# RQLuo/CDLNet-video

Hardware: AMD Instinct MI355X
Metric: Mpix/s denoised (fwd+bwd) at K=30,M=64,P=7 (higher is better)
Workload: dtype f32 (split-bf16 x3 MFMA, fp32 accumulate, fp32 storage)

## Files before the change

### cdlnet-video_amd/csrc/cdl_fused2d.hip

```cpp
#include <atomic>
#include <cstdlib>
#include <type_traits>
#include <mutex>
#include <utility>
#include <vector>

#include "cdl_common.h"

#ifdef CDL_F2D_WY4
#define CDL_WY 4
#define cdl_fused2d_assemble cdl_fused2d_assemble_wy4
#define cdl_fused2d_backward cdl_fused2d_backward_wy4
#define cdl_fused2d_code_bytes cdl_fused2d_code_bytes_wy4
#define cdl_fused2d_dtau_reduce cdl_fused2d_dtau_reduce_wy4
#define cdl_fused2d_forward cdl_fused2d_forward_wy4
#define cdl_fused2d_frag_bytes cdl_fused2d_frag_bytes_wy4
#define cdl_fused2d_iter_fwd cdl_fused2d_iter_fwd_wy4
#define cdl_fused2d_map_words cdl_fused2d_map_words_wy4
#define cdl_fused2d_patch_floats cdl_fused2d_patch_floats_wy4
#define cdl_fused2d_prep cdl_fused2d_prep_wy4
#define cdl_fused2d_stage_bwd cdl_fused2d_stage_bwd_wy4
#define cdl_fused2d_support_map cdl_fused2d_support_map_wy4
#define cdl_fused2d_supported cdl_fused2d_supported_wy4
#define cdl_fused2d_tiles cdl_fused2d_tiles_wy4
// ... 928 lines not shown
            ws |= (zz != 0.0f ? 1u : 0u) << (16 * R + v);
            wg |= (__builtin_bit_cast(unsigned, zz) >> 31) << (16 * R + v);
        }
    map[((size_t)n * 4 + 2 * h) * HW + pix] = ws;
    map[((size_t)n * 4 + 2 * h + 1) * HW + pix] = wg;
}

struct WgradParams {
    const float *X[2];
    const float *T[2];
    float *partial;
    int N, H, W, tilesX, tilesY, numTiles;
    int rev;
    int single;
};

template <int MT, int PREC, int LAY>
__global__ __launch_bounds__(512) void k_wgrad2d(WgradParams p)
{
    extern __shared__ __attribute__((aligned(16))) unsigned char dsm[];
    __bf16 *thin = reinterpret_cast<__bf16 *>(dsm);
    __bf16 *imgs = reinterpret_cast<__bf16 *>(dsm + WG_THIN_BYTES);
    constexpr int M = 32 * MT;
    const int tid = threadIdx.x, lane = tid & 63, wid = tid >> 6;
    const int op = wid >> 2, wq = wid & 3;
    const int wxi = wq & 1, wyi = wq >> 1;
    const int c = lane & 31, h = lane >> 5;
    const size_t HW = (size_t)p.H * p.W;
    __bf16 *wimg = imgs + (size_t)wid * (MT * 2) * IMG_ELEMS;
    f32x16 acc[MT][2];
#pragma unroll
    for (int R = 0; R < MT; ++R)
#pragma unroll
        for (int tt = 0; tt < 2; ++tt)
#pragma unroll
            for (int v = 0; v < 16; ++v) acc[R][tt][v] = 0.0f;

    for (int i = tid; i < WG_THIN_BYTES / 16; i += 512) reinterpret_cast<uint4 *>(dsm)[i] = make_uint4(0, 0, 0, 0);

    const bool present = p.X[op] != nullptr;
    const int nsteps = p.single ? (p.numTiles + 1) / 2 : p.numTiles;
    for (int t0 = blockIdx.x; t0 < nsteps; t0 += gridDim.x) {
        const int t = p.single ? 2 * t0 + op : t0;
        const bool active = present && t < p.numTiles;
        int bid = p.rev ? p.numTiles - 1 - t : t;
        const int txi = bid % p.tilesX; bid /= p.tilesX;
        const int tyi = bid % p.tilesY;
        const int n = active ? bid / p.tilesY : 0;
        const int tx0 = txi * TW, ty0 = tyi * GW_TH;
        __syncthreads();
        if (active) {
            const float *timg = p.T[op] + (size_t)n * HW;
            constexpr int NSW = (GW_RTH * RTW + 255) / 256;
            float tv[NSW];
#pragma unroll
            for (int k = 0; k < NSW; ++k) {
                const int i = (tid & 255) + k * 256;
                const int yy = i / RTW, xx = i % RTW;
                const int gy = ty0 - HALO + yy, gx = tx0 - HALO + xx;
                const bool ok = i < GW_RTH * RTW && gy >= 0 && gy < p.H && gx >= 0 && gx < p.W;
                const float v = timg[ok ? (size_t)gy * p.W + gx : 0];
                tv[k] = ok ? v : 0.0f;
            }
#pragma unroll
            for (int k = 0; k < NSW; ++k) {
                const int i = (tid & 255) + k * 256;
                if (i >= GW_RTH * RTW) continue;
                const int yy = i / RTW, xx = i % RTW;
                const __bf16 hh = (__bf16)tv[k];
                const __bf16 ll = (__bf16)(tv[k] - (float)hh);
#pragma unroll
                for (int s = 0; s < 4; ++s)
                    if (xx - s >= 0) {
                        thin[((op * 2 + 0) * 4 + s) * TCOPY + yy * TPITCH + xx - s] = hh;
                        if (PREC != 1) thin[((op * 2 + 1) * 4 + s) * TCOPY + yy * TPITCH + xx - s] = ll;
                    }
            }
        }
        __syncthreads();
        if (!active) continue;

        const int x = tx0 + wxi * 32 + c;
        const bool xok = x < p.W;
#pragma unroll 1
        for (int b = 0; b < RB; ++b) {
            const int yl = wyi * RB + b, y = ty0 + yl;
            const bool valid = xok && y < p.H;
            const size_t img_b = lay_image_bytes<LAY>(M, p.H, p.W);
            const __amdgpu_buffer_rsrc_t rs = uniform_rsrc((const char *)p.X[op] + (size_t)n * img_b, img_b);
            const int voff = valid ? (int)((4 * h) * HW + (size_t)y * p.W + x) * 4 : OOB;
            const int hw4 = (int)HW * 4;
            float xv[MT][16];
            u32x2 xr[MT][4];
            if (LAY == LAY_BLK16) {
                const int XB = (p.W + 31) / 32, xb = (tx0 >> 5) + wxi;
                blk16_load_raw<MT>(xr, rs, valid ? ((y * XB + xb) * (M / 4) * 32 + h * 32 + c) * 8 : OOB);
            } else if (LAY == LAY_BLK) {
                const int XB = (p.W + 31) / 32, xb = (tx0 >> 5) + wxi;
                blk_load<LAY_BLK, MT>(xv, rs, valid ? ((y * XB + xb) * (M / 4) * 32 + h * 32 + c) * 16 : OOB);
            } else {
#pragma unroll
                for (int R = 0; R < MT; ++R)
#pragma unroll
                    for (int v = 0; v < 16; ++v)
                        xv[R][v] = buf_ld(rs, voff, (32 * R + 8 * (v >> 2) + (v & 3)) * hw4);
            }
#pragma unroll
            for (int R = 0; R < MT; ++R)
#pragma unroll
                for (int qv = 0; qv < 4; ++qv) {
                    bf16x4 hi4, lo4;
                    if (LAY == LAY_BLK16) {
                        hi4 = __builtin_bit_cast(bf16x4, xr[R][qv]);
                    } else {
#pragma unroll
                        for (int e = 0; e < 4; ++e) {
                            const float val = xv[R][4 * qv + e];
                            const __bf16 hh = (__bf16)val;
                            hi4[e] = hh;
                            lo4[e] = (__bf16)(val - (float)hh);
                        }
                    }
                    const int slot = (2 * qv + h) ^ ((c >> 1) & 7);
                    __bf16 *dst = wimg + (size_t)(R * 2) * IMG_ELEMS + c * 32 + slot * 4;
                    *reinterpret_cast<bf16x4 *>(dst) = hi4;
                    if (PREC != 1 && LAY != LAY_BLK16) *reinterpret_cast<bf16x4 *>(dst + IMG_ELEMS) = lo4;
                }
            __builtin_amdgcn_fence(__ATOMIC_RELEASE, "wavefront");
            __builtin_amdgcn_wave_barrier();
#pragma unroll
            for (int kk = 0; kk < 2; ++kk) {
                bf16x8 Bh[2], Bl[2];
#pragma unroll
                for (int tt = 0; tt < 2; ++tt) {
                    const int tap = 32 * tt + c, ti = tap >> 3, tj = tap & 7;
                    const int e0 = wxi * 32 + 16 * kk + 8 * h + (tj & 4);
                    const __bf16 *ph = thin + ((op * 2 + 0) * 4 + (tj & 3)) * TCOPY + (yl + ti) * TPITCH + e0;
                    const bf16x4 a0 = *reinterpret_cast<const bf16x4 *>(ph);
                    const bf16x4 a1 = *reinterpret_cast<const bf16x4 *>(ph + 4);
                    Bh[tt] = __builtin_shufflevector(a0, a1, 0, 1, 2, 3, 4, 5, 6, 7);
                    if (PREC != 1) {
                        const __bf16 *pl = ph + 4 * TCOPY;
                        const bf16x4 b0 = *reinterpret_cast<const bf16x4 *>(pl);
                        const bf16x4 b1 = *reinterpret_cast<const bf16x4 *>(pl + 4);
                        Bl[tt] = __builtin_shufflevector(b0, b1, 0, 1, 2, 3, 4, 5, 6, 7);
                    }
                }
#pragma unroll
                for (int R = 0; R < MT; ++R) {
                    const int gg = (lane >> 4) & 1, qq = (lane >> 2) & 3, pp = lane & 3;
                    bf16x4 part[2][2];
#pragma unroll
                    for (int half = 0; half < 2; ++half) {
                        const int row = 16 * kk + 8 * h + 4 * half + qq;
                        const int slot = (4 * gg + pp) ^ ((row >> 1) & 7);
                        const __bf16 *src = wimg + (size_t)(R * 2) * IMG_ELEMS + row * 32 + slot * 4;
                        part[0][half] = __builtin_amdgcn_ds_read_tr16_b64_v4bf16(
                            (__attribute__((address_space(3))) bf16x4 *)(src));
                        if (PREC != 1 && LAY != LAY_BLK16)
                            part[1][half] = __builtin_amdgcn_ds_read_tr16_b64_v4bf16(
                                (__attribute__((address_space(3))) bf16x4 *)(src + IMG_ELEMS));
                    }
                    const bf16x8 Ah = __builtin_shufflevector(part[0][0], part[0][1], 0, 1, 2, 3, 4, 5, 6, 7);
                    bf16x8 Al;
                    if (PREC != 1 && LAY != LAY_BLK16) Al = __builtin_shufflevector(part[1][0], part[1][1], 0, 1, 2, 3, 4, 5, 6, 7);
#pragma unroll
                    for (int tt = 0; tt < 2; ++tt) {
                        if (PREC != 1) {
                            if (LAY != LAY_BLK16) acc[R][tt] = __builtin_amdgcn_mfma_f32_32x32x16_bf16(Al, Bh[tt], acc[R][tt], 0, 0, 0);
                            acc[R][tt] = __builtin_amdgcn_mfma_f32_32x32x16_bf16(Ah, Bl[tt], acc[R][tt], 0, 0, 0);
                            if (PREC == 2 && LAY != LAY_BLK16) acc[R][tt] = __builtin_amdgcn_mfma_f32_32x32x16_bf16(Al, Bl[tt], acc[R][tt], 0, 0, 0);
                        }
                        acc[R][tt] = __builtin_amdgcn_mfma_f32_32x32x16_bf16(Ah, Bh[tt], acc[R][tt], 0, 0, 0);
                    }
                }
            }
            __builtin_amdgcn_fence(__ATOMIC_RELEASE, "wavefront");
            __builtin_amdgcn_wave_barrier();
        }
    }

    float *red = reinterpret_cast<float *>(dsm);
    for (int w = 0; w < 4; ++w) {
        __syncthreads();
        if (wq == w) {
#pragma unroll
            for (int R = 0; R < MT; ++R)
#pragma unroll
                for (int tt = 0; tt < 2; ++tt)
#pragma unroll
                    for (int v = 0; v < 16; ++v) {
                        const int ch = 32 * R + (v & 3) + 8 * (v >> 2) + 4 * h;
                        float *dstw = &red[(op * M + ch) * 64 + 32 * tt + c];
                        *dstw = (w == 0 ? 0.0f : *dstw) + acc[R][tt][v];
                    }
        }
    }
    __syncthreads();
    float *dst = p.partial + (size_t)blockIdx.x * 2 * M * 64;
    for (int i = tid; i < 2 * M * 64; i += 512) dst[i] = red[i];
}

__global__ __launch_bounds__(1024) void k_wgrad_reduce(const float *__restrict__ partial, int G,
                                                       float *__restrict__ dw0, float alpha0,
                                                       float *__restrict__ dw1, float alpha1, int M, int P, int merge = 0)
{
    __shared__ float red[32][33];
    const int o = threadIdx.x & 31, part = threadIdx.x >> 5;
    const int t = blockIdx.x * 32 + o;
    const int per = M * P * P;
    const bool live = t < (merge ? per : 2 * per);
    float sum = 0.0f;
    int op = 0, r = 0;
    if (live) {
        op = t / per; r = t % per;
        const int ch = r / (P * P), ij = r % (P * P), off = (7 - P) / 2;
        const int tap = 8 * (ij / P + off) + (ij % P + off);
        for (int g = part; g < G; g += 32) {
            sum += partial[((size_t)(g * 2 + op) * M + ch) * 64 + tap];
            if (merge) sum += partial[((size_t)(g * 2 + 1) * M + ch) * 64 + tap];
        }
    }
    red[part][o] = sum;
    __syncthreads();
    if (part == 0 && live) {
        float *dw = op ? dw1 : dw0;
        if (dw) {
            float tot = 0.0f;
#pragma unroll
            for (int k = 0; k < 32; ++k) tot += red[k][o];
            dw[r] = (op ? alpha1 : alpha0) * tot;
        }
    }
}

__global__ __launch_bounds__(1024) void k_dtau_reduce(const float *__restrict__ partial,
                                                      const float *__restrict__ c, float *__restrict__ dt0,
                                                      float *__restrict__ dt1, int N, int per_img, int M)
{
    __shared__ float r0[256][4], r1[256][4];
    const int mi = threadIdx.x & 3, part = threadIdx.x >> 2;
    const int m = blockIdx.x * 4 + mi;
    float a0 = 0.0f, a1 = 0.0f;
    const int rows = N * per_img;
    if (m < M)
        for (int row = part; row < rows; row += 256) {
            const float v = partial[(size_t)row * M + m];
            a0 += v;
            if (c) a1 = fmaf(c[row / per_img], v, a1);
        }
    r0[part][mi] = a0;
    r1[part][mi] = a1;
    __syncthreads();
    for (int stride = 128; stride >= 1; stride >>= 1) {
        if (part < stride) { r0[part][mi] += r0[part + stride][mi]; r1[part][mi] += r1[part + stride][mi]; }
        __syncthreads();
    }
    if (part == 0 && m < M) { dt0[m] = r0[0][mi]; dt1[m] = r1[0][mi]; }
}

inline hipStream_t S(void *s) { return reinterpret_cast<hipStream_t>(s); }

inline bool fused_shape_ok(const cdl_geom *g)
{
    if (!cdl_geom_ok(g)) return false;
    if (g->C != 1 || g->D != 1 || g->Pd != 1 || g->sd != 1 || g->sh != 1 || g->sw != 1) return false;
    if (g->Ph != g->Pw || g->Ph > 7 || (g->Ph & 1) == 0 || g->ph != g->Ph / 2 || g->pw != g->Pw / 2) return false;
    if (g->M != 32 && g->M != 64) return false;
    if (blk_image_elems(g->M, g->H, g->W) * 4 >= ((size_t)1 << 31)) return false;
    return true;
}

inline int debug_flags() { return cdl_opts().fused_debug; }

inline int tiles_x(const cdl_geom *g) { return (g->W + TW - 1) / TW; }
inline int tiles_y(const cdl_geom *g) { return (g->H + TH - 1) / TH; }

struct Flags {
    int prec, rev, lin, lout;
    bool ok;
};
// ... 58 lines not shown
{
    const size_t tiles = (size_t)p.N * p.tilesX * p.tilesY;
    size_t cus = (size_t)cdl_cu_count();
    const int cap = cdl_opts().fused_grid;
    if (cap > 0 && (size_t)cap < cus) cus = (size_t)cap;
    return (int)(tiles < cus ? tiles : cus);
}

int dispatch_stage(const cdl_geom *g, const FusedParams &p, int mode, const Flags &f, hipStream_t st)
{
    dim3 grid((unsigned)stage_grid(g, p));
    if (g->M == 64)
        return f.prec == 0   ? launch_stage<2, 0>(p, mode, f.lin, f.lout, grid, st)
               : f.prec == 1 ? launch_stage<2, 1>(p, mode, f.lin, f.lout, grid, st)
                             : launch_stage<2, 2>(p, mode, f.lin, f.lout, grid, st);
    return f.prec == 0   ? launch_stage<1, 0>(p, mode, f.lin, f.lout, grid, st)
           : f.prec == 1 ? launch_stage<1, 1>(p, mode, f.lin, f.lout, grid, st)
                         : launch_stage<1, 2>(p, mode, f.lin, f.lout, grid, st);
}

int wgrad_grid(const cdl_geom *g)
{
    const size_t tiles = (size_t)g->N * tiles_x(g) * ((g->H + GW_TH - 1) / GW_TH);
    return (int)(tiles < 512 ? tiles : 512);
}

template <int MT, int PREC, int LAY>
int launch_wgrad_one(const WgradParams &p, int G, hipStream_t st)
{
    const size_t lds = (size_t)WG_THIN_BYTES + (size_t)8 * MT * 2 * IMG_ELEMS * 2;
    if (int rc = cdl_ensure_dynamic_lds((const void *)k_wgrad2d<MT, PREC, LAY>, (int)lds)) return rc;
    k_wgrad2d<MT, PREC, LAY><<<G, 512, lds, st>>>(p);
    hipError_t e = hipGetLastError();
    return e == hipSuccess ? 0 : -(int)e;
}

template <int MT, int PREC>
int launch_wgrad(const WgradParams &p, int lay, int G, hipStream_t st)
{
    if (lay == LAY_BLK) return launch_wgrad_one<MT, PREC, LAY_BLK>(p, G, st);
    if (lay == LAY_BLK16) return launch_wgrad_one<MT, PREC, LAY_BLK16>(p, G, st);
    return launch_wgrad_one<MT, PREC, LAY_NCHW>(p, G, st);
}

}

extern "C" {

// ... 64 lines not shown
    k_support_map<<<(unsigned)((total + 255) / 256), 256, 0, S(stream)>>>(z, map, g->N, g->M, g->H, g->W);
    CDL_LAUNCH_CHECK();
    return 0;
}

int cdl_fused2d_iter_fwd(const cdl_geom *g, const float *r, const float *zin, const float *tau,
                         const void *frags, float sgn, float *zout, float *patches, unsigned *map_out,
                         int precision, void *stream)
{
    if (!fused_shape_ok(g)) return CDL_EUNSUPPORTED;
    if (!r || !tau || !frags || !zout || !patches || zout == zin) return CDL_EINVAL;
    const Flags f = parse_flags(precision);
    if (!f.ok) return CDL_EINVAL;
    FusedParams p = {};
    p.rev = f.rev;
    p.r = r; p.zin = zin; p.zout = zout; p.tau = tau; p.map = map_out;
    p.frags = reinterpret_cast<const uint4 *>(frags);
    p.patches = patches; p.sgn = sgn; p.do_synth = 1; CDL_DBG_FIELD(p.dbg = debug_flags();)
    p.N = g->N; p.H = g->H; p.W = g->W;
    p.tilesX = tiles_x(g); p.tilesY = tiles_y(g);
    return dispatch_stage(g, p, zin ? MODE_FWD : MODE_FIRST, f, S(stream));
}

static int stage_bwd(const cdl_geom *g, const float *thin, const float *base, const unsigned *map, const void *frags,
                     float *du_out, float *patches, float *dtau_partial, int do_synth, int precision, const float *r2,
                     float alpha, float *dA, float *workspace, void *stream)
{
    if (!fused_shape_ok(g)) return CDL_EUNSUPPORTED;
    if (!thin || !map || !frags || !du_out || !dtau_partial || du_out == base) return CDL_EINVAL;
    if (do_synth && !patches) return CDL_EINVAL;
    if (r2 && (!dA || !workspace)) return CDL_EINVAL;
    const Flags f = parse_flags(precision);
    if (!f.ok) return CDL_EINVAL;
    FusedParams p = {};
    p.rev = f.rev;
    p.r = thin; p.zin = base; p.map = const_cast<unsigned *>(map); p.zout = du_out; p.dtau = dtau_partial;
    p.frags = reinterpret_cast<const uint4 *>(frags);
    p.patches = patches; p.sgn = 1.0f; p.do_synth = do_synth ? 1 : 0; CDL_DBG_FIELD(p.dbg = debug_flags();)
    p.N = g->N; p.H = g->H; p.W = g->W;
    p.tilesX = tiles_x(g); p.tilesY = tiles_y(g);
    p.r2 = r2; p.da_partial = workspace;
    int rc = dispatch_stage(g, p, MODE_BWD, f, S(stream));
    if (rc || !r2) return rc;
    const int G = stage_grid(g, p);
    const int total = 2 * g->M * g->Ph * g->Pw;
    k_wgrad_reduce<<<(total + 31) / 32, 1024, 0, S(stream)>>>(workspace, G, dA, alpha, nullptr, 0.0f, g->M, g->Ph);
    CDL_LAUNCH_CHECK();
    return 0;
}

int cdl_fused2d_stage_bwd(const cdl_geom *g, const float *thin, const float *base, const unsigned *map,
                          const void *frags, float *du_out, float *patches, float *dtau_partial, int do_synth,
                          const float *r2, float alpha, float *dA, float *workspace, int precision, void *stream)
{
    if (!r2 != !dA || !r2 != !workspace) return CDL_EINVAL;
    return stage_bwd(g, thin, base, map, frags, du_out, patches, dtau_partial, do_synth, precision, r2, alpha, dA, workspace,
                     stream);
}

int cdl_fused2d_dtau_reduce(const cdl_geom *g, const float *dtau_partial, const float *c, float *dt0, float *dt1,
                            float *dtau_n, void *stream)
{
    if (!fused_shape_ok(g)) return CDL_EUNSUPPORTED;
    if (!dtau_partial || !dt0 || !dt1) return CDL_EINVAL;
    const int per_img = tiles_x(g) * tiles_y(g);
    k_dtau_reduce<<<(g->M + 3) / 4, 1024, 0, S(stream)>>>(dtau_partial, c, dt0, dt1, g->N, per_img, g->M);
    CDL_LAUNCH_CHECK();
    if (!dtau_n) return 0;
    return cdl_dtau_per_sample(dtau_partial, g->N, g->M, per_img, (size_t)per_img * g->M, 1, g->M, dtau_n, stream);
}

size_t cdl_fused2d_wgrad_workspace_floats(const cdl_geom *g)
{
    if (!fused_shape_ok(g)) return 0;
    const size_t own = (size_t)wgrad_grid(g) * 2 * g->M * 64;
#ifndef CDL_F2D_WY4
    return larger(own, cdl_fused2d_wgrad_workspace_floats_wy4(g));
#else
    return own;
#endif
}

int cdl_fused2d_wgrad(const cdl_geom *g, const float *X0, const float *T0, float alpha0, float *dw0,
                      const float *X1, const float *T1, float alpha1, float *dw1, float *workspace,
                      int precision, void *stream)
{
    if (!fused_shape_ok(g)) return CDL_EUNSUPPORTED;
    if (!workspace || (!X0 && !X1)) return CDL_EINVAL;
    if ((X0 && (!T0 || !dw0)) || (X1 && (!T1 || !dw1))) return CDL_EINVAL;
    const Flags f = parse_flags(precision);
    if (!f.ok) return CDL_EINVAL;
    WgradParams p = {};
    p.rev = f.rev;
    p.X[0] = X0; p.T[0] = T0; p.X[1] = X1; p.T[1] = T1;
    p.single = (X0 != nullptr) != (X1 != nullptr);
    if (p.single) {
        if (!X0) { X0 = X1; T0 = T1; alpha0 = alpha1; dw0 = dw1; X1 = nullptr; }
        p.X[0] = p.X[1] = X0; p.T[0] = p.T[1] = T0;
    }
    p.partial = workspace;
    p.N = g->N; p.H = g->H; p.W = g->W;
    p.tilesX = tiles_x(g); p.tilesY = (g->H + GW_TH - 1) / GW_TH;
    p.numTiles = p.N * p.tilesX * p.tilesY;
    int G = wgrad_grid(g);
    if (p.single && G > (p.numTiles + 1) / 2) G = (p.numTiles + 1) / 2;
    int rc;
    if (g->M == 64)
        rc = f.prec == 0 ? launch_wgrad<2, 0>(p, f.lin, G, S(stream))
             : f.prec == 1 ? launch_wgrad<2, 1>(p, f.lin, G, S(stream)) : launch_wgrad<2, 2>(p, f.lin, G, S(stream));
    else
        rc = f.prec == 0 ? launch_wgrad<1, 0>(p, f.lin, G, S(stream))
             : f.prec == 1 ? launch_wgrad<1, 1>(p, f.lin, G, S(stream)) : launch_wgrad<1, 2>(p, f.lin, G, S(stream));
    if (rc) return rc;
    const int total = 2 * g->M * g->Ph * g->Pw;
    k_wgrad_reduce<<<(total + 31) / 32, 1024, 0, S(stream)>>>(workspace, G, X0 ? dw0 : nullptr, alpha0,
                                                             X1 ? dw1 : nullptr, alpha1, g->M, g->Ph, p.single);
    CDL_LAUNCH_CHECK();
    return 0;
}

int cdl_fused2d_assemble(const cdl_geom *g, const float *patches, const float *mask, const float *sub,
                         float alpha, float *out, float *acc, int acc_add, void *stream)
{
    if (!fused_shape_ok(g)) return CDL_EUNSUPPORTED;
    if (!patches || (!out && !acc)) return CDL_EINVAL;
    if ((size_t)g->N * g->H * g->W >= ((size_t)1 << 20) && (g->W & 3) == 0 && !cdl_opts().scalar_assemble) {
        dim3 grid((unsigned)((g->W + 255) / 256), (unsigned)((g->H + 7) / 8), (unsigned)g->N);
        k_assemble_v4<<<grid, 256, 0, S(stream)>>>(patches, mask, sub, alpha, out, g->N, g->H, g->W, tiles_x(g), tiles_y(g), acc, acc_add);
    } else if ((size_t)g->N * g->H * g->W >= ((size_t)1 << 20)) {
        dim3 grid((unsigned)((g->W + 255) / 256), (unsigned)((g->H + 3) / 4), (unsigned)g->N);
        k_assemble<4><<<grid, 256, 0, S(stream)>>>(patches, mask, sub, alpha, out, g->N, g->H, g->W, tiles_x(g), tiles_y(g), acc, acc_add);
    } else {
        dim3 grid((unsigned)((g->W + 255) / 256), (unsigned)g->H, (unsigned)g->N);
        k_assemble<1><<<grid, 256, 0, S(stream)>>>(patches, mask, sub, alpha, out, g->N, g->H, g->W, tiles_x(g), tiles_y(g), acc, acc_add);
    }
    CDL_LAUNCH_CHECK();
    return 0;
}

}

// ... 170 lines not shown
    if (K < 1 || !yp || !wA || !wB || !z || !maps || !g_xp || !dA || !dB || !dt || !du0 || !du1 || !q || !frags ||
        !patches || !dtau_partial || !wgrad_ws || (K > 1 && !r))
        return CDL_EINVAL;
    const int M = g->M;
    float *du[2] = {du0, du1};
    const Flags f = parse_flags(precision);
    if (!f.ok || f.lout != 0) return CDL_EINVAL;
    const int L = f.lin;
#ifndef CDL_F2D_WY4
    if (L == LAY_BLK16)
        return cdl_fused2d_backward_wy4(g, K, yp, mask, c, wA, wB, z, r, maps, g_xp, g_z, dA, dB, dt, du0, du1, q, frags,
                                        patches, dtau_partial, wgrad_ws, precision, dyp, dtau, stream);
#endif
    const int sdir = snake_enabled() ? (((K - 1) & 1) ? CDL_TILES_REVERSED : 0) : 0;
    const int wdir = snake_enabled() ? (sdir ^ CDL_TILES_REVERSED) : 0;
    const int sprec = f.prec | sdir, wprec = f.prec | wdir;
    int rc = cdl_fused2d_wgrad(g, z[K - 1], g_xp, 1.0f, dB[0], nullptr, nullptr, 0.0f, nullptr, wgrad_ws,
                               wprec, stream);
    if (rc) return rc;
    const float *thin = g_xp, *base = g_z;
    const size_t fb = cdl_fused2d_frag_bytes(M);
    rc = prep_pairs(wB, wA, K, 0, frags, M, g->Ph, S(stream));
    if (rc) return rc;
    for (int k = K - 1, flip = 0; k >= 0; --k, flip ^= 1) {
        const void *fk = static_cast<const char *>(frags) + (size_t)k * fb;
        float *duk = du[flip];
        const bool ride = TH == GW_TH && cdl_opts().fused_da;
        {
            TimingScope ts(1, S(stream));
            rc = stage_bwd(g, thin, base, maps[k], fk, duk, patches, dtau_partial, k >= 1 || dyp,
                           sprec | CDL_LAYOUT_IN(k == K - 1 ? LAY_NCHW : L) | CDL_LAYOUT_OUT(L),
                           ride ? (k >= 1 ? r[k - 1] : yp) : nullptr, k >= 1 ? -1.0f : 1.0f, dA[k], wgrad_ws, stream);
        }
        if (rc) return rc;
        rc = cdl_fused2d_dtau_reduce(g, dtau_partial, c, dt + (size_t)k * 2 * M, dt + (size_t)k * 2 * M + M,
                                     dtau ? dtau + (size_t)k * g->N * M : nullptr, stream);
        if (rc) return rc;
        if (k == 0 && dyp) {
            rc = cdl_fused2d_assemble(g, patches, nullptr, nullptr, 1.0f, nullptr, dyp, K > 1, stream);
            if (rc) return rc;
        }
        if (k >= 1) {
            rc = cdl_fused2d_assemble(g, patches, mask, nullptr, -1.0f, q, dyp, k < K - 1, stream);
            if (rc) return rc;
            {
                TimingScope ts(2, S(stream));
                rc = ride ? cdl_fused2d_wgrad(g, z[k - 1], q, 1.0f, dB[k], nullptr, nullptr, 0.0f, nullptr, wgrad_ws,
                                              wprec | CDL_LAYOUT_IN(L), stream)
                          : cdl_fused2d_wgrad(g, duk, r[k - 1], -1.0f, dA[k], z[k - 1], q, 1.0f, dB[k], wgrad_ws,
                                              wprec | CDL_LAYOUT_IN(L), stream);
            }
            thin = q;
        } else if (!ride) {
            rc = cdl_fused2d_wgrad(g, duk, yp, 1.0f, dA[0], nullptr, nullptr, 0.0f, nullptr, wgrad_ws,
                                   wprec | CDL_LAYOUT_IN(L), stream);
        }
        if (rc) return rc;
        base = duk;
    }
    return 0;
}

}
```

### cdlnet-video_amd/ops.py

```python
import ctypes
from dataclasses import dataclass
from typing import Optional, Tuple

import torch

from . import _lib


def _stream():
    return ctypes.c_void_p(torch.cuda.current_stream().cuda_stream)


def _first_cuda_tensor(args, kwargs=None):
    for a in list(args) + (list(kwargs.values()) if kwargs else []):
        if torch.is_tensor(a):
            if a.is_cuda:
                return a
        elif isinstance(a, (list, tuple)):
            t = _first_cuda_tensor(a)
            if t is not None:
                return t
    return None


# ... 626 lines not shown
                                          float(alpha), _ptr(dA), _ptr(workspace), flags, _stream())
    _lib.check(rc, "cdl_fused2d_stage_bwd")
    return out if dA is None else (out, dA)


def fused_dtau_reduce(g: Geometry, dtau_partial, c, dt_k, dtau_n=None):
    assert dt_k.is_contiguous() and dt_k.numel() == 2 * g.M
    assert dtau_n is None or (dtau_n.is_contiguous() and dtau_n.numel() == g.N * g.M)
    gs = g.c_struct()
    base = dt_k.data_ptr()
    rc = _lib.lib().cdl_fused2d_dtau_reduce(ctypes.byref(gs), _ptr(dtau_partial), _ptr(_opt(c, "c")),
                                            ctypes.c_void_p(base), ctypes.c_void_p(base + 4 * g.M), _ptr(dtau_n),
                                            _stream())
    _lib.check(rc, "cdl_fused2d_dtau_reduce")


def fused_wgrad_workspace(g: Geometry, device):
    gs = g.c_struct()
    n = _lib.lib().cdl_fused2d_wgrad_workspace_floats(ctypes.byref(gs))
    return torch.empty(n, device=device, dtype=torch.float32)


def fused_wgrad(g: Geometry, workspace, X0=None, T0=None, alpha0=1.0, X1=None, T1=None, alpha1=1.0,
                precision="split3", layout="nchw"):
    outs = []
    args = []
    for X, T, al in ((X0, T0, alpha0), (X1, T1, alpha1)):
        if X is None:
            outs.append(None)
            args += [None, None, 0.0, None]
        else:
            X, T = (_dev(X, "X") if layout == "nchw" else X), _dev(T, "T")
            dw = torch.empty(g.filter_shape(), device=X.device, dtype=torch.float32)
            outs.append(dw)
            args += [_ptr(X), _ptr(T), float(al), _ptr(dw)]
    gs = g.c_struct()
    rc = _lib.lib().cdl_fused2d_wgrad(ctypes.byref(gs), *args, _ptr(workspace),
                                      PRECISION[precision] | _lay_in(layout), _stream())
    _lib.check(rc, "cdl_fused2d_wgrad")
    return outs


def _check_data_grads(g: Geometry, K, dyp, dtau):
    for t, shape in ((dyp, g.image_shape()), (dtau, (K, g.N, g.M))):
        if t is not None:
            assert t.is_cuda and t.dtype == torch.float32 and t.is_contiguous() and tuple(t.shape) == tuple(shape), \
                (tuple(t.shape), shape)


def _ptr_table(tensors):
    return (ctypes.c_void_p * len(tensors))(*[t.data_ptr() for t in tensors])


def fused_forward(g: Geometry, yp, mask_p, tau, A, B, keep, precision="split3", layout="blocked"):
    K = len(A)
    yp, tau = _dev(yp, "yp"), _dev(tau, "tau")
    mask_p = _opt(mask_p, "mask")
    A = [_dev(w, "A") for w in A]
    B = [_dev(w, "B") for w in B]
    dev = yp.device
    nz = (K - 1) if keep else min(K - 1, 2)
# ... 342 lines not shown
```

Measured before the change: 118.4.

## Double-buffer wgrad row loads and merge per-stage reductions into one sweep launch

```diff
diff --git a/cdlnet-video_amd/csrc/cdl_fused2d.hip b/cdlnet-video_amd/csrc/cdl_fused2d.hip
--- a/cdlnet-video_amd/csrc/cdl_fused2d.hip
+++ b/cdlnet-video_amd/csrc/cdl_fused2d.hip
@@ -974,7 +974,7 @@
     __bf16 *thin = reinterpret_cast<__bf16 *>(dsm);
     __bf16 *imgs = reinterpret_cast<__bf16 *>(dsm + WG_THIN_BYTES);
     constexpr int M = 32 * MT;
-    const int tid = threadIdx.x, lane = tid & 63, wid = tid >> 6;
+    const int tid = threadIdx.x, lane = tid & 63, wid = __builtin_amdgcn_readfirstlane(tid >> 6);
     const int op = wid >> 2, wq = wid & 3;
     const int wxi = wq & 1, wyi = wq >> 1;
     const int c = lane & 31, h = lane >> 5;
@@ -992,144 +992,171 @@
 
     const bool present = p.X[op] != nullptr;
     const int nsteps = p.single ? (p.numTiles + 1) / 2 : p.numTiles;
-    for (int t0 = blockIdx.x; t0 < nsteps; t0 += gridDim.x) {
+    const size_t img_b = lay_image_bytes<LAY>(M, p.H, p.W);
+    const int hw4 = (int)HW * 4;
+
+    struct Tile { bool active; int n, tx0, ty0; };
+    auto tile_at = [&](int t0) {
         const int t = p.single ? 2 * t0 + op : t0;
-        const bool active = present && t < p.numTiles;
+        Tile q;
+        q.active = present && t0 < nsteps && t < p.numTiles;
         int bid = p.rev ? p.numTiles - 1 - t : t;
         const int txi = bid % p.tilesX; bid /= p.tilesX;
         const int tyi = bid % p.tilesY;
-        const int n = active ? bid / p.tilesY : 0;
-        const int tx0 = txi * TW, ty0 = tyi * GW_TH;
-        __syncthreads();
-        if (active) {
-            const float *timg = p.T[op] + (size_t)n * HW;
-            constexpr int NSW = (GW_RTH * RTW + 255) / 256;
-            float tv[NSW];
-#pragma unroll
-            for (int k = 0; k < NSW; ++k) {
-                const int i = (tid & 255) + k * 256;
-                const int yy = i / RTW, xx = i % RTW;
-                const int gy = ty0 - HALO + yy, gx = tx0 - HALO + xx;
-                const bool ok = i < GW_RTH * RTW && gy >= 0 && gy < p.H && gx >= 0 && gx < p.W;
-                const float v = timg[ok ? (size_t)gy * p.W + gx : 0];
-                tv[k] = ok ? v : 0.0f;
-            }
-#pragma unroll
-            for (int k = 0; k < NSW; ++k) {
-                const int i = (tid & 255) + k * 256;
-                if (i >= GW_RTH * RTW) continue;
-                const int yy = i / RTW, xx = i % RTW;
-                const __bf16 hh = (__bf16)tv[k];
-                const __bf16 ll = (__bf16)(tv[k] - (float)hh);
-#pragma unroll
-                for (int s = 0; s < 4; ++s)
-                    if (xx - s >= 0) {
-                        thin[((op * 2 + 0) * 4 + s) * TCOPY + yy * TPITCH + xx - s] = hh;
-                        if (PREC != 1) thin[((op * 2 + 1) * 4 + s) * TCOPY + yy * TPITCH + xx - s] = ll;
-                    }
-            }
-        }
-        __syncthreads();
-        if (!active) continue;
-
-        const int x = tx0 + wxi * 32 + c;
-        const bool xok = x < p.W;
-#pragma unroll 1
-        for (int b = 0; b < RB; ++b) {
-            const int yl = wyi * RB + b, y = ty0 + yl;
-            const bool valid = xok && y < p.H;
-            const size_t img_b = lay_image_bytes<LAY>(M, p.H, p.W);
-            const __amdgpu_buffer_rsrc_t rs = uniform_rsrc((const char *)p.X[op] + (size_t)n * img_b, img_b);
+        q.n = q.active ? bid / p.tilesY : 0;
+        q.tx0 = txi * TW; q.ty0 = tyi * GW_TH;
+        return q;
+    };
+    constexpr int NSW = (GW_RTH * RTW + 255) / 256;
+    auto thin_load = [&](float (&tv)[NSW], const Tile &q) {
+        const float *timg = p.T[op] + (size_t)q.n * HW;
+#pragma unroll
+        for (int k = 0; k < NSW; ++k) {
+            const int i = (tid & 255) + k * 256;
+            const int yy = i / RTW, xx = i % RTW;
+            const int gy = q.ty0 - HALO + yy, gx = q.tx0 - HALO + xx;
+            const bool ok = i < GW_RTH * RTW && gy >= 0 && gy < p.H && gx >= 0 && gx < p.W;
+            const float v = timg[ok ? (size_t)gy * p.W + gx : 0];
+            tv[k] = ok ? v : 0.0f;
+        }
+    };
+    auto thin_write = [&](const float (&tv)[NSW]) {
+#pragma unroll
+        for (int k = 0; k < NSW; ++k) {
+            const int i = (tid & 255) + k * 256;
+            if (i >= GW_RTH * RTW) continue;
+            const int yy = i / RTW, xx = i % RTW;
+            const __bf16 hh = (__bf16)tv[k];
+            const __bf16 ll = (__bf16)(tv[k] - (float)hh);
+#pragma unroll
+            for (int s = 0; s < 4; ++s)
+                if (xx - s >= 0) {
+                    thin[((op * 2 + 0) * 4 + s) * TCOPY + yy * TPITCH + xx - s] = hh;
+                    if (PREC != 1) thin[((op * 2 + 1) * 4 + s) * TCOPY + yy * TPITCH + xx - s] = ll;
+                }
+        }
+    };
+    struct Fat {
+        float xv[MT][16];
+        u32x2 xr[MT][4];
+    };
+    auto fat_load = [&](Fat &f, const Tile &q, int b) {
+        const int x = q.tx0 + wxi * 32 + c, y = q.ty0 + wyi * RB + b;
+        const bool valid = q.active && x < p.W && y < p.H;
+        const __amdgpu_buffer_rsrc_t rs = uniform_rsrc((const char *)p.X[op] + (size_t)q.n * img_b, img_b);
+        if (LAY == LAY_BLK16) {
+            const int XB = (p.W + 31) / 32, xb = (q.tx0 >> 5) + wxi;
+            blk16_load_raw<MT>(f.xr, rs, valid ? ((y * XB + xb) * (M / 4) * 32 + h * 32 + c) * 8 : OOB);
+        } else if (LAY == LAY_BLK) {
+            const int XB = (p.W + 31) / 32, xb = (q.tx0 >> 5) + wxi;
+            blk_load<LAY_BLK, MT>(f.xv, rs, valid ? ((y * XB + xb) * (M / 4) * 32 + h * 32 + c) * 16 : OOB);
+        } else {
             const int voff = valid ? (int)((4 * h) * HW + (size_t)y * p.W + x) * 4 : OOB;
-            const int hw4 = (int)HW * 4;
-            float xv[MT][16];
-            u32x2 xr[MT][4];
-            if (LAY == LAY_BLK16) {
-                const int XB = (p.W + 31) / 32, xb = (tx0 >> 5) + wxi;
-                blk16_load_raw<MT>(xr, rs, valid ? ((y * XB + xb) * (M / 4) * 32 + h * 32 + c) * 8 : OOB);
-            } else if (LAY == LAY_BLK) {
-                const int XB = (p.W + 31) / 32, xb = (tx0 >> 5) + wxi;
-                blk_load<LAY_BLK, MT>(xv, rs, valid ? ((y * XB + xb) * (M / 4) * 32 + h * 32 + c) * 16 : OOB);
-            } else {
-#pragma unroll
-                for (int R = 0; R < MT; ++R)
-#pragma unroll
-                    for (int v = 0; v < 16; ++v)
-                        xv[R][v] = buf_ld(rs, voff, (32 * R + 8 * (v >> 2) + (v & 3)) * hw4);
-            }
 #pragma unroll
             for (int R = 0; R < MT; ++R)
 #pragma unroll
-                for (int qv = 0; qv < 4; ++qv) {
-                    bf16x4 hi4, lo4;
-                    if (LAY == LAY_BLK16) {
-                        hi4 = __builtin_bit_cast(bf16x4, xr[R][qv]);
-                    } else {
-#pragma unroll
-                        for (int e = 0; e < 4; ++e) {
-                            const float val = xv[R][4 * qv + e];
-                            const __bf16 hh = (__bf16)val;
-                            hi4[e] = hh;
-                            lo4[e] = (__bf16)(val - (float)hh);
-                        }
-                    }
-                    const int slot = (2 * qv + h) ^ ((c >> 1) & 7);
-                    __bf16 *dst = wimg + (size_t)(R * 2) * IMG_ELEMS + c * 32 + slot * 4;
-                    *reinterpret_cast<bf16x4 *>(dst) = hi4;
-                    if (PREC != 1 && LAY != LAY_BLK16) *reinterpret_cast<bf16x4 *>(dst + IMG_ELEMS) = lo4;
-                }
-            __builtin_amdgcn_fence(__ATOMIC_RELEASE, "wavefront");
-            __builtin_amdgcn_wave_barrier();
-#pragma unroll
-            for (int kk = 0; kk < 2; ++kk) {
-                bf16x8 Bh[2], Bl[2];
-#pragma unroll
-                for (int tt = 0; tt < 2; ++tt) {
-                    const int tap = 32 * tt + c, ti = tap >> 3, tj = tap & 7;
-                    const int e0 = wxi * 32 + 16 * kk + 8 * h + (tj & 4);
-                    const __bf16 *ph = thin + ((op * 2 + 0) * 4 + (tj & 3)) * TCOPY + (yl + ti) * TPITCH + e0;
-                    const bf16x4 a0 = *reinterpret_cast<const bf16x4 *>(ph);
-                    const bf16x4 a1 = *reinterpret_cast<const bf16x4 *>(ph + 4);
-                    Bh[tt] = __builtin_shufflevector(a0, a1, 0, 1, 2, 3, 4, 5, 6, 7);
-                    if (PREC != 1) {
-                        const __bf16 *pl = ph + 4 * TCOPY;
-                        const bf16x4 b0 = *reinterpret_cast<const bf16x4 *>(pl);
-                        const bf16x4 b1 = *reinterpret_cast<const bf16x4 *>(pl + 4);
-                        Bl[tt] = __builtin_shufflevector(b0, b1, 0, 1, 2, 3, 4, 5, 6, 7);
+                for (int v = 0; v < 16; ++v)
+                    f.xv[R][v] = buf_ld(rs, voff, (32 * R + 8 * (v >> 2) + (v & 3)) * hw4);
+        }
+    };
+    auto row_block = [&](const Fat &f, int b) {
+        const int yl = wyi * RB + b;
+#pragma unroll
+        for (int R = 0; R < MT; ++R)
+#pragma unroll
+            for (int qv = 0; qv < 4; ++qv) {
+                bf16x4 hi4, lo4;
+                if (LAY == LAY_BLK16) {
+                    hi4 = __builtin_bit_cast(bf16x4, f.xr[R][qv]);
+                } else {
+#pragma unroll
+                    for (int e = 0; e < 4; ++e) {
+                        const float val = f.xv[R][4 * qv + e];
+                        const __bf16 hh = (__bf16)val;
+                        hi4[e] = hh;
+                        lo4[e] = (__bf16)(val - (float)hh);
                     }
                 }
-#pragma unroll
-                for (int R = 0; R < MT; ++R) {
-                    const int gg = (lane >> 4) & 1, qq = (lane >> 2) & 3, pp = lane & 3;
-                    bf16x4 part[2][2];
-#pragma unroll
-                    for (int half = 0; half < 2; ++half) {
-                        const int row = 16 * kk + 8 * h + 4 * half + qq;
-                        const int slot = (4 * gg + pp) ^ ((row >> 1) & 7);
-                        const __bf16 *src = wimg + (size_t)(R * 2) * IMG_ELEMS + row * 32 + slot * 4;
-                        part[0][half] = __builtin_amdgcn_ds_read_tr16_b64_v4bf16(
-                            (__attribute__((address_space(3))) bf16x4 *)(src));
-                        if (PREC != 1 && LAY != LAY_BLK16)
-                            part[1][half] = __builtin_amdgcn_ds_read_tr16_b64_v4bf16(
-                                (__attribute__((address_space(3))) bf16x4 *)(src + IMG_ELEMS));
-                    }
-                    const bf16x8 Ah = __builtin_shufflevector(part[0][0], part[0][1], 0, 1, 2, 3, 4, 5, 6, 7);
-                    bf16x8 Al;
-                    if (PREC != 1 && LAY != LAY_BLK16) Al = __builtin_shufflevector(part[1][0], part[1][1], 0, 1, 2, 3, 4, 5, 6, 7);
-#pragma unroll
-                    for (int tt = 0; tt < 2; ++tt) {
-                        if (PREC != 1) {
-                            if (LAY != LAY_BLK16) acc[R][tt] = __builtin_amdgcn_mfma_f32_32x32x16_bf16(Al, Bh[tt], acc[R][tt], 0, 0, 0);
-                            acc[R][tt] = __builtin_amdgcn_mfma_f32_32x32x16_bf16(Ah, Bl[tt], acc[R][tt], 0, 0, 0);
-                            if (PREC == 2 && LAY != LAY_BLK16) acc[R][tt] = __builtin_amdgcn_mfma_f32_32x32x16_bf16(Al, Bl[tt], acc[R][tt], 0, 0, 0);
-                        }
-                        acc[R][tt] = __builtin_amdgcn_mfma_f32_32x32x16_bf16(Ah, Bh[tt], acc[R][tt], 0, 0, 0);
-                    }
+                const int slot = (2 * qv + h) ^ ((c >> 1) & 7);
+                __bf16 *dst = wimg + (size_t)(R * 2) * IMG_ELEMS + c * 32 + slot * 4;
+                *reinterpret_cast<bf16x4 *>(dst) = hi4;
+                if (PREC != 1 && LAY != LAY_BLK16) *reinterpret_cast<bf16x4 *>(dst + IMG_ELEMS) = lo4;
+            }
+        __builtin_amdgcn_fence(__ATOMIC_RELEASE, "wavefront");
+        __builtin_amdgcn_wave_barrier();
+#pragma unroll
+        for (int kk = 0; kk < 2; ++kk) {
+            bf16x8 Bh[2], Bl[2];
+#pragma unroll
+            for (int tt = 0; tt < 2; ++tt) {
+                const int tap = 32 * tt + c, ti = tap >> 3, tj = tap & 7;
+                const int e0 = wxi * 32 + 16 * kk + 8 * h + (tj & 4);
+                const __bf16 *ph = thin + ((op * 2 + 0) * 4 + (tj & 3)) * TCOPY + (yl + ti) * TPITCH + e0;
+                const bf16x4 a0 = *reinterpret_cast<const bf16x4 *>(ph);
+                const bf16x4 a1 = *reinterpret_cast<const bf16x4 *>(ph + 4);
+                Bh[tt] = __builtin_shufflevector(a0, a1, 0, 1, 2, 3, 4, 5, 6, 7);
+                if (PREC != 1) {
+                    const __bf16 *pl = ph + 4 * TCOPY;
+                    const bf16x4 b0 = *reinterpret_cast<const bf16x4 *>(pl);
+                    const bf16x4 b1 = *reinterpret_cast<const bf16x4 *>(pl + 4);
+                    Bl[tt] = __builtin_shufflevector(b0, b1, 0, 1, 2, 3, 4, 5, 6, 7);
                 }
             }
-            __builtin_amdgcn_fence(__ATOMIC_RELEASE, "wavefront");
-            __builtin_amdgcn_wave_barrier();
-        }
+#pragma unroll
+            for (int R = 0; R < MT; ++R) {
+                const int gg = (lane >> 4) & 1, qq = (lane >> 2) & 3, pp = lane & 3;
+                bf16x4 part[2][2];
+#pragma unroll
+                for (int half = 0; half < 2; ++half) {
+                    const int row = 16 * kk + 8 * h + 4 * half + qq;
+                    const int slot = (4 * gg + pp) ^ ((row >> 1) & 7);
+                    const __bf16 *src = wimg + (size_t)(R * 2) * IMG_ELEMS + row * 32 + slot * 4;
+                    part[0][half] = __builtin_amdgcn_ds_read_tr16_b64_v4bf16(
+                        (__attribute__((address_space(3))) bf16x4 *)(src));
+                    if (PREC != 1 && LAY != LAY_BLK16)
+                        part[1][half] = __builtin_amdgcn_ds_read_tr16_b64_v4bf16(
+                            (__attribute__((address_space(3))) bf16x4 *)(src + IMG_ELEMS));
+                }
+                const bf16x8 Ah = __builtin_shufflevector(part[0][0], part[0][1], 0, 1, 2, 3, 4, 5, 6, 7);
+                bf16x8 Al;
+                if (PREC != 1 && LAY != LAY_BLK16) Al = __builtin_shufflevector(part[1][0], part[1][1], 0, 1, 2, 3, 4, 5, 6, 7);
+#pragma unroll
+                for (int tt = 0; tt < 2; ++tt) {
+                    if (PREC != 1) {
+                        if (LAY != LAY_BLK16) acc[R][tt] = __builtin_amdgcn_mfma_f32_32x32x16_bf16(Al, Bh[tt], acc[R][tt], 0, 0, 0);
+                        acc[R][tt] = __builtin_amdgcn_mfma_f32_32x32x16_bf16(Ah, Bl[tt], acc[R][tt], 0, 0, 0);
+                        if (PREC == 2 && LAY != LAY_BLK16) acc[R][tt] = __builtin_amdgcn_mfma_f32_32x32x16_bf16(Al, Bl[tt], acc[R][tt], 0, 0, 0);
+                    }
+                    acc[R][tt] = __builtin_amdgcn_mfma_f32_32x32x16_bf16(Ah, Bh[tt], acc[R][tt], 0, 0, 0);
+                }
+            }
+        }
+        __builtin_amdgcn_fence(__ATOMIC_RELEASE, "wavefront");
+        __builtin_amdgcn_wave_barrier();
+    };
+
+    static_assert(RB % 2 == 0, "the row loop alternates between two landing sets");
+    Tile cur = tile_at(blockIdx.x);
+    Fat fa, fb;
+    fat_load(fa, cur, 0);
+    for (int t0 = blockIdx.x; t0 < nsteps; t0 += gridDim.x) {
+        const Tile nxt = tile_at(t0 + gridDim.x);
+        __syncthreads();
+        if (cur.active) {
+            float tv[NSW];
+            thin_load(tv, cur);
+            thin_write(tv);
+        }
+        __syncthreads();
+#pragma unroll 1
+        for (int b = 0; b < RB; b += 2) {
+            fat_load(fb, cur, b + 1);
+            if (cur.active) row_block(fa, b);
+            if (b + 2 < RB) fat_load(fa, cur, b + 2);
+            else fat_load(fa, nxt, 0);
+            if (cur.active) row_block(fb, b + 1);
+        }
+        cur = nxt;
     }
 
     float *red = reinterpret_cast<float *>(dsm);
@@ -1153,53 +1180,70 @@
     for (int i = tid; i < 2 * M * 64; i += 512) dst[i] = red[i];
 }
 
-__global__ __launch_bounds__(1024) void k_wgrad_reduce(const float *__restrict__ partial, int G,
-                                                       float *__restrict__ dw0, float alpha0,
-                                                       float *__restrict__ dw1, float alpha1, int M, int P, int merge = 0)
-{
-    __shared__ float red[32][33];
+struct WgradReduce {
+    const float *partial;
+    int G;
+    float *dw0, *dw1;
+    float alpha0, alpha1;
+    int merge;
+};
+__device__ __forceinline__ void wgrad_reduce_block(float (*red)[33], int block, const WgradReduce &q, int M, int P)
+{
+    const float *__restrict__ partial = q.partial;
     const int o = threadIdx.x & 31, part = threadIdx.x >> 5;
-    const int t = blockIdx.x * 32 + o;
+    const int t = block * 32 + o;
     const int per = M * P * P;
-    const bool live = t < (merge ? per : 2 * per);
+    const bool live = t < (q.merge ? per : 2 * per);
     float sum = 0.0f;
     int op = 0, r = 0;
     if (live) {
         op = t / per; r = t % per;
         const int ch = r / (P * P), ij = r % (P * P), off = (7 - P) / 2;
         const int tap = 8 * (ij / P + off) + (ij % P + off);
-        for (int g = part; g < G; g += 32) {
+        for (int g = part; g < q.G; g += 32) {
             sum += partial[((size_t)(g * 2 + op) * M + ch) * 64 + tap];
-            if (merge) sum += partial[((size_t)(g * 2 + 1) * M + ch) * 64 + tap];
+            if (q.merge) sum += partial[((size_t)(g * 2 + 1) * M + ch) * 64 + tap];
         }
     }
     red[part][o] = sum;
     __syncthreads();
     if (part == 0 && live) {
-        float *dw = op ? dw1 : dw0;
+        float *dw = op ? q.dw1 : q.dw0;
         if (dw) {
             float tot = 0.0f;
 #pragma unroll
             for (int k = 0; k < 32; ++k) tot += red[k][o];
-            dw[r] = (op ? alpha1 : alpha0) * tot;
-        }
-    }
-}
-
-__global__ __launch_bounds__(1024) void k_dtau_reduce(const float *__restrict__ partial,
-                                                      const float *__restrict__ c, float *__restrict__ dt0,
-                                                      float *__restrict__ dt1, int N, int per_img, int M)
-{
-    __shared__ float r0[256][4], r1[256][4];
+            dw[r] = (op ? q.alpha1 : q.alpha0) * tot;
+        }
+    }
+}
+inline int wgrad_reduce_blocks(const WgradReduce &q, int M, int P) { return ((q.merge ? 1 : 2) * M * P * P + 31) / 32; }
+
+__global__ __launch_bounds__(1024) void k_wgrad_reduce(WgradReduce q, int M, int P)
+{
+    __shared__ float red[32][33];
+    wgrad_reduce_block(red, blockIdx.x, q, M, P);
+}
+
+struct DtauReduce {
+    const float *partial;
+    const float *c;
+    float *dt0, *dt1;
+    int N, per_img;
+};
+__device__ __forceinline__ void dtau_reduce_block(float (*r0)[4], float (*r1)[4], int block, const DtauReduce &q, int M)
+{
+    const float *__restrict__ partial = q.partial;
+    const float *__restrict__ c = q.c;
     const int mi = threadIdx.x & 3, part = threadIdx.x >> 2;
-    const int m = blockIdx.x * 4 + mi;
+    const int m = block * 4 + mi;
     float a0 = 0.0f, a1 = 0.0f;
-    const int rows = N * per_img;
+    const int rows = q.N * q.per_img;
     if (m < M)
         for (int row = part; row < rows; row += 256) {
             const float v = partial[(size_t)row * M + m];
             a0 += v;
-            if (c) a1 = fmaf(c[row / per_img], v, a1);
+            if (c) a1 = fmaf(c[row / q.per_img], v, a1);
         }
     r0[part][mi] = a0;
     r1[part][mi] = a1;
@@ -1208,7 +1252,34 @@
         if (part < stride) { r0[part][mi] += r0[part + stride][mi]; r1[part][mi] += r1[part + stride][mi]; }
         __syncthreads();
     }
-    if (part == 0 && m < M) { dt0[m] = r0[0][mi]; dt1[m] = r1[0][mi]; }
+    if (part == 0 && m < M) { q.dt0[m] = r0[0][mi]; q.dt1[m] = r1[0][mi]; }
+}
+
+__global__ __launch_bounds__(1024) void k_dtau_reduce(DtauReduce q, int M)
+{
+    __shared__ float r0[256][4], r1[256][4];
+    dtau_reduce_block(r0, r1, blockIdx.x, q, M);
+}
+
+struct SweepReduce {
+    WgradReduce w[2];
+    int wblocks[2];
+    DtauReduce t;
+};
+__global__ __launch_bounds__(1024) void k_sweep_reduce(SweepReduce q, int M, int P)
+{
+    __shared__ float sm[2 * 256 * 4];
+    static_assert(sizeof(sm) >= 32 * 33 * sizeof(float), "k_wgrad_reduce's staging fits too");
+    int block = blockIdx.x;
+#pragma unroll
+    for (int j = 0; j < 2; ++j) {
+        if (block < q.wblocks[j]) {
+            wgrad_reduce_block(reinterpret_cast<float (*)[33]>(sm), block, q.w[j], M, P);
+            return;
+        }
+        block -= q.wblocks[j];
+    }
+    dtau_reduce_block(reinterpret_cast<float (*)[4]>(sm), reinterpret_cast<float (*)[4]>(sm + 256 * 4), block, q.t, M);
 }
 
 inline hipStream_t S(void *s) { return reinterpret_cast<hipStream_t>(s); }
@@ -1313,8 +1384,11 @@
 int wgrad_grid(const cdl_geom *g)
 {
     const size_t tiles = (size_t)g->N * tiles_x(g) * ((g->H + GW_TH - 1) / GW_TH);
-    return (int)(tiles < 512 ? tiles : 512);
-}
+    const size_t cus = (size_t)cdl_cu_count();
+    return (int)(tiles < cus ? tiles : cus);
+}
+
+size_t wgrad_region_floats(const cdl_geom *g) { return (size_t)wgrad_grid(g) * 2 * g->M * 64; }
 
 template <int MT, int PREC, int LAY>
 int launch_wgrad_one(const WgradParams &p, int G, hipStream_t st)
@@ -1425,9 +1499,16 @@
     return dispatch_stage(g, p, zin ? MODE_FWD : MODE_FIRST, f, S(stream));
 }
 
+static int launch_wgrad_reduce(const cdl_geom *g, const WgradReduce &job, hipStream_t st)
+{
+    k_wgrad_reduce<<<wgrad_reduce_blocks(job, g->M, g->Ph), 1024, 0, st>>>(job, g->M, g->Ph);
+    hipError_t e = hipGetLastError();
+    return e == hipSuccess ? 0 : -(int)e;
+}
+
 static int stage_bwd(const cdl_geom *g, const float *thin, const float *base, const unsigned *map, const void *frags,
                      float *du_out, float *patches, float *dtau_partial, int do_synth, int precision, const float *r2,
-                     float alpha, float *dA, float *workspace, void *stream)
+                     float alpha, float *dA, float *workspace, void *stream, WgradReduce *defer = nullptr)
 {
     if (!fused_shape_ok(g)) return CDL_EUNSUPPORTED;
     if (!thin || !map || !frags || !du_out || !dtau_partial || du_out == base) return CDL_EINVAL;
@@ -1445,11 +1526,9 @@
     p.r2 = r2; p.da_partial = workspace;
     int rc = dispatch_stage(g, p, MODE_BWD, f, S(stream));
     if (rc || !r2) return rc;
-    const int G = stage_grid(g, p);
-    const int total = 2 * g->M * g->Ph * g->Pw;
-    k_wgrad_reduce<<<(total + 31) / 32, 1024, 0, S(stream)>>>(workspace, G, dA, alpha, nullptr, 0.0f, g->M, g->Ph);
-    CDL_LAUNCH_CHECK();
-    return 0;
+    const WgradReduce job = {workspace, stage_grid(g, p), dA, nullptr, alpha, 0.0f, 0};
+    if (defer) { *defer = job; return 0; }
+    return launch_wgrad_reduce(g, job, S(stream));
 }
 
 int cdl_fused2d_stage_bwd(const cdl_geom *g, const float *thin, const float *base, const unsigned *map,
@@ -1467,7 +1546,8 @@
     if (!fused_shape_ok(g)) return CDL_EUNSUPPORTED;
     if (!dtau_partial || !dt0 || !dt1) return CDL_EINVAL;
     const int per_img = tiles_x(g) * tiles_y(g);
-    k_dtau_reduce<<<(g->M + 3) / 4, 1024, 0, S(stream)>>>(dtau_partial, c, dt0, dt1, g->N, per_img, g->M);
+    const DtauReduce job = {dtau_partial, c, dt0, dt1, g->N, per_img};
+    k_dtau_reduce<<<(g->M + 3) / 4, 1024, 0, S(stream)>>>(job, g->M);
     CDL_LAUNCH_CHECK();
     if (!dtau_n) return 0;
     return cdl_dtau_per_sample(dtau_partial, g->N, g->M, per_img, (size_t)per_img * g->M, 1, g->M, dtau_n, stream);
@@ -1476,7 +1556,7 @@
 size_t cdl_fused2d_wgrad_workspace_floats(const cdl_geom *g)
 {
     if (!fused_shape_ok(g)) return 0;
-    const size_t own = (size_t)wgrad_grid(g) * 2 * g->M * 64;
+    const size_t own = 2 * wgrad_region_floats(g);
 #ifndef CDL_F2D_WY4
     return larger(own, cdl_fused2d_wgrad_workspace_floats_wy4(g));
 #else
@@ -1484,9 +1564,9 @@
 #endif
 }
 
-int cdl_fused2d_wgrad(const cdl_geom *g, const float *X0, const float *T0, float alpha0, float *dw0,
-                      const float *X1, const float *T1, float alpha1, float *dw1, float *workspace,
-                      int precision, void *stream)
+static int wgrad_partials(const cdl_geom *g, const float *X0, const float *T0, float alpha0, float *dw0,
+                          const float *X1, const float *T1, float alpha1, float *dw1, float *workspace,
+                          int precision, void *stream, WgradReduce *job)
 {
     if (!fused_shape_ok(g)) return CDL_EUNSUPPORTED;
     if (!workspace || (!X0 && !X1)) return CDL_EINVAL;
@@ -1515,11 +1595,17 @@
         rc = f.prec == 0 ? launch_wgrad<1, 0>(p, f.lin, G, S(stream))
              : f.prec == 1 ? launch_wgrad<1, 1>(p, f.lin, G, S(stream)) : launch_wgrad<1, 2>(p, f.lin, G, S(stream));
     if (rc) return rc;
-    const int total = 2 * g->M * g->Ph * g->Pw;
-    k_wgrad_reduce<<<(total + 31) / 32, 1024, 0, S(stream)>>>(workspace, G, X0 ? dw0 : nullptr, alpha0,
-                                                             X1 ? dw1 : nullptr, alpha1, g->M, g->Ph, p.single);
-    CDL_LAUNCH_CHECK();
+    *job = WgradReduce{workspace, G, X0 ? dw0 : nullptr, X1 ? dw1 : nullptr, alpha0, alpha1, p.single};
     return 0;
+}
+
+int cdl_fused2d_wgrad(const cdl_geom *g, const float *X0, const float *T0, float alpha0, float *dw0,
+                      const float *X1, const float *T1, float alpha1, float *dw1, float *workspace,
+                      int precision, void *stream)
+{
+    WgradReduce job;
+    if (int rc = wgrad_partials(g, X0, T0, alpha0, dw0, X1, T1, alpha1, dw1, workspace, precision, stream, &job)) return rc;
+    return launch_wgrad_reduce(g, job, S(stream));
 }
 
 int cdl_fused2d_assemble(const cdl_geom *g, const float *patches, const float *mask, const float *sub,
@@ -1736,20 +1822,26 @@
     const size_t fb = cdl_fused2d_frag_bytes(M);
     rc = prep_pairs(wB, wA, K, 0, frags, M, g->Ph, S(stream));
     if (rc) return rc;
+    float *ws_a = wgrad_ws, *ws_b = wgrad_ws + wgrad_region_floats(g);
+    const int per_img = tiles_x(g) * tiles_y(g);
     for (int k = K - 1, flip = 0; k >= 0; --k, flip ^= 1) {
         const void *fk = static_cast<const char *>(frags) + (size_t)k * fb;
         float *duk = du[flip];
         const bool ride = TH == GW_TH && cdl_opts().fused_da;
+        SweepReduce red = {};
         {
             TimingScope ts(1, S(stream));
             rc = stage_bwd(g, thin, base, maps[k], fk, duk, patches, dtau_partial, k >= 1 || dyp,
                            sprec | CDL_LAYOUT_IN(k == K - 1 ? LAY_NCHW : L) | CDL_LAYOUT_OUT(L),
-                           ride ? (k >= 1 ? r[k - 1] : yp) : nullptr, k >= 1 ? -1.0f : 1.0f, dA[k], wgrad_ws, stream);
+                           ride ? (k >= 1 ? r[k - 1] : yp) : nullptr, k >= 1 ? -1.0f : 1.0f, dA[k], ws_a, stream, &red.w[0]);
         }
         if (rc) return rc;
-        rc = cdl_fused2d_dtau_reduce(g, dtau_partial, c, dt + (size_t)k * 2 * M, dt + (size_t)k * 2 * M + M,
-                                     dtau ? dtau + (size_t)k * g->N * M : nullptr, stream);
-        if (rc) return rc;
+        if (ride) red.wblocks[0] = wgrad_reduce_blocks(red.w[0], M, g->Ph);
+        red.t = DtauReduce{dtau_partial, c, dt + (size_t)k * 2 * M, dt + (size_t)k * 2 * M + M, g->N, per_img};
+        if (dtau) {
+            rc = cdl_dtau_per_sample(dtau_partial, g->N, M, per_img, (size_t)per_img * M, 1, M, dtau + (size_t)k * g->N * M, stream);
+            if (rc) return rc;
+        }
         if (k == 0 && dyp) {
             rc = cdl_fused2d_assemble(g, patches, nullptr, nullptr, 1.0f, nullptr, dyp, K > 1, stream);
             if (rc) return rc;
@@ -1759,17 +1851,20 @@
             if (rc) return rc;
             {
                 TimingScope ts(2, S(stream));
-                rc = ride ? cdl_fused2d_wgrad(g, z[k - 1], q, 1.0f, dB[k], nullptr, nullptr, 0.0f, nullptr, wgrad_ws,
-                                              wprec | CDL_LAYOUT_IN(L), stream)
-                          : cdl_fused2d_wgrad(g, duk, r[k - 1], -1.0f, dA[k], z[k - 1], q, 1.0f, dB[k], wgrad_ws,
-                                              wprec | CDL_LAYOUT_IN(L), stream);
+                rc = ride ? wgrad_partials(g, z[k - 1], q, 1.0f, dB[k], nullptr, nullptr, 0.0f, nullptr, ws_b,
+                                           wprec | CDL_LAYOUT_IN(L), stream, &red.w[1])
+                          : wgrad_partials(g, duk, r[k - 1], -1.0f, dA[k], z[k - 1], q, 1.0f, dB[k], ws_b,
+                                           wprec | CDL_LAYOUT_IN(L), stream, &red.w[1]);
             }
             thin = q;
         } else if (!ride) {
-            rc = cdl_fused2d_wgrad(g, duk, yp, 1.0f, dA[0], nullptr, nullptr, 0.0f, nullptr, wgrad_ws,
-                                   wprec | CDL_LAYOUT_IN(L), stream);
+            rc = wgrad_partials(g, duk, yp, 1.0f, dA[0], nullptr, nullptr, 0.0f, nullptr, ws_b, wprec | CDL_LAYOUT_IN(L), stream,
+                                &red.w[1]);
         }
         if (rc) return rc;
+        if (k >= 1 || !ride) red.wblocks[1] = wgrad_reduce_blocks(red.w[1], M, g->Ph);
+        k_sweep_reduce<<<red.wblocks[0] + red.wblocks[1] + (M + 3) / 4, 1024, 0, S(stream)>>>(red, M, g->Ph);
+        CDL_LAUNCH_CHECK();
         base = duk;
     }
     return 0;
diff --git a/cdlnet-video_amd/ops.py b/cdlnet-video_amd/ops.py
--- a/cdlnet-video_amd/ops.py
+++ b/cdlnet-video_amd/ops.py
@@ -672,7 +672,7 @@
 
 
 def fused_wgrad(g: Geometry, workspace, X0=None, T0=None, alpha0=1.0, X1=None, T1=None, alpha1=1.0,
-                precision="split3", layout="nchw"):
+                precision="split3", layout="nchw", tiles_reversed=False):
     outs = []
     args = []
     for X, T, al in ((X0, T0, alpha0), (X1, T1, alpha1)):
@@ -686,7 +686,8 @@
             args += [_ptr(X), _ptr(T), float(al), _ptr(dw)]
     gs = g.c_struct()
     rc = _lib.lib().cdl_fused2d_wgrad(ctypes.byref(gs), *args, _ptr(workspace),
-                                      PRECISION[precision] | _lay_in(layout), _stream())
+                                      PRECISION[precision] | _lay_in(layout) | (TILES_REVERSED if tiles_reversed else 0),
+                                      _stream())
     _lib.check(rc, "cdl_fused2d_wgrad")
     return outs
 
```

Result: faster. 121.3, median of 6 (+2.4%).
